# LMCache/LMCache

Hardware: NVIDIA B200
Metric: kv_encode_decode_raw_GBps (higher is better)
Workload: dtype f32->u8 (bf16 KV)

## Files before the change

lmcache_b200/csrc/codec.cu:

```cuda
#include <cuda_bf16.h>
#include <cuda_fp16.h>
#include <cuda_runtime.h>
#include <stdint.h>
#include <stdlib.h>

#include "ac_core.cuh"
#include "common.cuh"

namespace b200kv {

constexpr int CT = 128;
constexpr int SPW = 6;
constexpr int SYMW = 43;
constexpr int PAIRW = 33;
constexpr int TEMPW_FUSED = 40;
constexpr int TEMPW_SPLIT = 132;
constexpr int TEMPW_FUSED_RANS = 48;
constexpr int CODER_AC = 0, CODER_RANS = 1;
constexpr int CODER_RANS_COMPACT = 2;
constexpr int kHdrRowWords = 8;
constexpr int TEMPW_FUSED_RANS_HDR = TEMPW_FUSED_RANS + kHdrRowWords;

struct EncParams {
    PlaneTable pt;
    int64_t sT, sH, tok_begin;
    const int64_t* slot_map;
    int32_t L, H, D, C, dtype;
    int32_t n_chunks, chunk_tokens, last_chunk_tokens, tpp;
    int32_t tiles_full, tempw;
    int32_t stage_bytes;
    int32_t coder;
    int32_t compact;
    uint8_t* out;
    int64_t out_stride;
    uint64_t* sizes_out;
    uint32_t* temp;
    uint32_t* rstate;
    uint32_t* tile_tot;
    unsigned long long* totals;
    unsigned int* err;
};

template <class Prm>
__device__ __forceinline__ Layout layout_of(const Prm& P, int t) {
    return make_layout(P.L, P.C, t, P.compact);
}

__device__ __forceinline__ uint32_t load_len(const uint8_t* sec, int64_t idx, bool compact) {
    return compact ? 2u * (uint32_t)sec[idx] : (uint32_t)reinterpret_cast<const int32_t*>(sec)[idx];
}
__device__ __forceinline__ void store_len(uint8_t* sec, int64_t idx, uint32_t len, bool compact) {
    if (compact) sec[idx] = (uint8_t)(len >> 1);
    else reinterpret_cast<int32_t*>(sec)[idx] = (int32_t)len;
}

__device__ __forceinline__ uint32_t build_stream_header(const uint32_t (&cnt)[32], uint32_t mask, uint32_t wany, int nb,
                                                        uint32_t* rowfront, uint32_t& w0, uint32_t& w1) {
    const uint32_t top = 0x80000000u >> __clz((int)mask);
    const uint32_t st = mask & ~top;
    const uint32_t mb = (uint32_t)hdr_mask_bytes(nb);
    w0 = 0u;
    w1 = 0u;
    uint32_t widx = 0u, acc = mask, sh = 8u * mb;
    auto flush = [&]() {
        if (widx == 0u) w0 = acc;
        else if (widx == 1u) w1 = acc;
        else rowfront[widx - 2u] = acc;
        ++widx;
        acc = 0u;
        sh = 0u;
    };
    if (sh == 32u) flush();
#pragma unroll
    for (int i = 0; i < 32; ++i) {
        if (i < nb && ((wany >> i) & 1u) && ((st >> i) & 1u)) {
            acc |= cnt[i] << sh;
            sh += 8u;
            if (sh == 32u) flush();
        }
    }
    uint32_t hlen = mb + (uint32_t)__popc(st);
    hlen += hlen & 1u;
    if (sh != 0u) flush();
    return hlen;
}

__device__ __forceinline__ uint32_t read_header_mask(const uint8_t* p, int nb) {
    uint32_t m = *reinterpret_cast<const uint16_t*>(p);
    if (nb > 16) m |= (uint32_t)*reinterpret_cast<const uint16_t*>(p + 2) << 16;
    if (nb <= 8) m &= 0xffu;
    return nb >= 32 ? m : m & ((1u << nb) - 1u);
}

__device__ __forceinline__ int chunk_tokens_of(const EncParams& P, int j) {
    return j == P.n_chunks - 1 ? P.last_chunk_tokens : P.chunk_tokens;
}

template <bool PAGED>
__device__ __forceinline__ int64_t tok_row(const int64_t* slot_map, int64_t tok) {
    if constexpr (PAGED) return __ldg(slot_map + tok);
    else return tok;
}

template <bool VEC, bool PAGED>
__global__ void __launch_bounds__(256) absmax_kernel(EncParams P, int64_t total_tokens) {
    const int64_t warp = (blockIdx.x * (int64_t)blockDim.x + threadIdx.x) >> 5;
    const int lane = threadIdx.x & 31;
    const int64_t nrows = (int64_t)2 * P.L * total_tokens;
    if (warp >= nrows) return;
    const int nl = (int)(warp / total_tokens);
    const int64_t T = warp % total_tokens;
    const uint16_t* row = P.pt.p[nl] + tok_row<PAGED>(P.slot_map, P.tok_begin + T) * P.sT;
    uint32_t m = 0;
    if (VEC) {
        const int vec_per_head = P.D >> 3;
        const int nvec = P.H * vec_per_head;
        for (int v = lane; v < nvec; v += 32) {
            const int h = v / vec_per_head, dv = v - h * vec_per_head;
            const uint4 q = __ldg(reinterpret_cast<const uint4*>(row + (int64_t)h * P.sH + dv * 8));
            const uint32_t w[4] = {q.x, q.y, q.z, q.w};
#pragma unroll
            for (int k = 0; k < 4; ++k) {
                const uint32_t a = w[k] & 0x7fff7fffu;
                m = max(m, max(a & 0xffffu, a >> 16));
            }
        }
    } else {
        for (int c = lane; c < P.C; c += 32) {
            const int h = c / P.D, d = c - h * P.D;
            m = max(m, (uint32_t)(__ldg(row + (int64_t)h * P.sH + d) & 0x7fffu));
        }
    }
    m = __reduce_max_sync(0xffffffffu, m);
    if (lane == 0) {
        const int j = (int)(T / P.chunk_tokens);
        const int tj = chunk_tokens_of(P, j);
        const Layout lo = layout_of(P, tj);
        uint16_t* maxes = reinterpret_cast<uint16_t*>(P.out + (int64_t)j * P.out_stride + lo.off_maxes);
        maxes[(int64_t)nl * tj + (T - (int64_t)j * P.chunk_tokens)] = (uint16_t)m;
    }
}

__device__ __forceinline__ uint32_t block_excl_scan(uint32_t v, uint32_t* s_warp, uint32_t* total) {
    const int lane = threadIdx.x & 31, wid = threadIdx.x >> 5;
    uint32_t inc = v;
#pragma unroll
    for (int o = 1; o < 32; o <<= 1) {
        uint32_t n = __shfl_up_sync(0xffffffffu, inc, o);
        if (lane >= o) inc += n;
    }
    if (lane == 31) s_warp[wid] = inc;
    __syncthreads();
    uint32_t base = 0, tot = 0;
#pragma unroll
    for (int w = 0; w < CT / 32; ++w) {
        const uint32_t s = s_warp[w];
        if (w < wid) base += s;
        tot += s;
    }
    *total = tot;
    return base + inc - v;
}

struct TileId { int j, g, nl, ct, t, tok0, gt, tile_in_chunk; };
__device__ __forceinline__ bool decode_tile(const EncParams& P, uint32_t tile, TileId* id) {
    const uint32_t per_group = 2u * P.L * P.tpp;
    const uint32_t j = tile / (uint32_t)P.tiles_full;
    const uint32_t rem = tile - j * (uint32_t)P.tiles_full;
    id->j = (int)j;
    id->tile_in_chunk = (int)rem;
    id->t = chunk_tokens_of(P, (int)j);
    id->g = (int)(rem / per_group);
    if (id->g * kGroup >= id->t) return false;
    const uint32_t rem2 = rem - (uint32_t)id->g * per_group;
    id->nl = (int)(rem2 / P.tpp);
    id->ct = (int)(rem2 - (uint32_t)id->nl * P.tpp);
    id->tok0 = id->g * kGroup;
    id->gt = min(kGroup, id->t - id->tok0);
    return true;
}

template <int DT, bool PAGED, int BT, class F>
__device__ __forceinline__ void for_each_symbol(const uint16_t* cbase, const int64_t* slot_map, int64_t tokabs, int64_t s1,
                                                int gt, const float* fac, float maxq, F&& f) {
    const int nbatch = (gt + BT - 1) / BT;
    uint16_t xa[BT], xb[BT];
    auto load = [&](uint16_t (&x)[BT], int b) {
        const int tk = b * BT;
#pragma unroll
        for (int k = 0; k < BT; ++k)
            x[k] = tk + k < gt ? __ldg(cbase + tok_row<PAGED>(slot_map, tokabs + tk + k) * s1) : (uint16_t)0;
    };
    auto use = [&](const uint16_t (&x)[BT], int b) {
        const int tk = b * BT;
        uint32_t q[BT];
#pragma unroll
        for (int k = 0; k < BT; ++k) q[k] = quant_symbol(half_to_float(x[k], DT), fac[min(tk + k, kGroup - 1)], maxq);
#pragma unroll
        for (int k = 0; k < BT; ++k)
            if (tk + k < gt) f(q[k]);
    };
    load(xa, 0);
    for (int b = 0; b < nbatch; b += 2) {
        if (b + 1 < nbatch) load(xb, b + 1);
        use(xa, b);
        if (b + 1 < nbatch) {
            if (b + 2 < nbatch) load(xa, b + 2);
            use(xb, b + 1);
        }
    }
}

template <int DT, bool PAGED, int BT, class F>
__device__ __forceinline__ void for_each_symbol_rev(const uint16_t* cbase, const int64_t* slot_map, int64_t tokabs, int64_t s1,
                                                    int gt, const float* fac, float maxq, F&& f) {
    const int nbatch = (gt + BT - 1) / BT;
    uint16_t xa[BT], xb[BT];
    auto load = [&](uint16_t (&x)[BT], int b) {
        const int tk = b * BT;
#pragma unroll
        for (int k = 0; k < BT; ++k)
            x[k] = tk + k < gt ? __ldg(cbase + tok_row<PAGED>(slot_map, tokabs + tk + k) * s1) : (uint16_t)0;
    };
    auto use = [&](const uint16_t (&x)[BT], int b) {
        const int tk = b * BT;
        uint32_t q[BT];
#pragma unroll
        for (int k = 0; k < BT; ++k) q[k] = quant_symbol(half_to_float(x[k], DT), fac[min(tk + k, kGroup - 1)], maxq);
#pragma unroll
        for (int k = BT - 1; k >= 0; --k)
            if (tk + k < gt) f(q[k]);
    };
    load(xa, nbatch - 1);
    for (int b = nbatch - 1; b >= 0; b -= 2) {
        if (b >= 1) load(xb, b - 1);
        use(xa, b);
        if (b >= 1) {
            if (b >= 2) load(xa, b - 2);
            use(xb, b - 1);
        }
    }
}

__device__ __forceinline__ void rans_put(uint32_t& x, int32_t& nk, const uint16_t* row_end, uint32_t start, uint32_t freq) {
    const uint32_t xh = x >> 16;
    asm volatile(
        "{\n\t.reg .pred p;\n\t.reg .b64 ad;\n\t"
        "setp.ge.u32 p, %2, %3;\n\t"
        "mad.wide.s32 ad, %1, 2, %4;\n\t"
        "@p st.global.u16 [ad+-2], %0;\n\t"
        "@p add.s32 %1, %1, -1;\n\t"
        "selp.b32 %0, %2, %0, p;\n\t"
        "}"
        : "+r"(x), "+r"(nk) : "r"(xh), "r"(freq), "l"(row_end) : "memory");
    float rc;
    asm("rcp.approx.ftz.f32 %0, %1;" : "=f"(rc) : "f"(__uint2float_rn(freq)));
    const uint32_t q = __float2uint_rz(__uint2float_rz(x) * (rc * 0.99999952316284179688f));
    const uint32_t m = 65536u - freq;
    const uint32_t a = q * m + x;
    const uint32_t r = a - (q << 16);
    x = a + start;
    if (r >= freq) x += m;
}

template <bool FUSED, int DT, bool PAGED, int CODER>
__global__ void __launch_bounds__(CT, FUSED ? 7 : 4) encode_kernel(EncParams P) {
    extern __shared__ __align__(16) uint32_t smem[];
    constexpr int ROWS_W = FUSED ? CT * SYMW : 0;
    constexpr int TAB_W = FUSED ? (CT * kLp * 2 + 3) / 4 : CT * PAIRW;
    uint32_t* rows = smem;
    uint32_t* tab = smem + ROWS_W;
    float* fac = reinterpret_cast<float*>(smem + ((ROWS_W + TAB_W + 3) & ~3));
    __shared__ uint32_t s_warp[CT / 32];

    const int tid = threadIdx.x;
    TileId id;
    if (!decode_tile(P, blockIdx.x, &id)) return;
    const int NL = 2 * P.L;
    const int j = id.j, nl = id.nl, ct = id.ct, t = id.t, gt = id.gt;
    const int c = ct * CT + tid;
    const bool active = c < P.C;
    const int ncols = min(CT, P.C - ct * CT);

    uint8_t* cont = P.out + (int64_t)j * P.out_stride;
    const Layout lo = layout_of(P, t);
    const uint16_t* maxes = reinterpret_cast<const uint16_t*>(cont + lo.off_maxes) + (int64_t)nl * t + id.tok0;
    const float maxq = P.pt.maxq[nl];
    const int64_t s1 = P.sT;
    for (int i = tid; i < gt; i += CT)
        fac[i] = FUSED ? quant_factor_safe(maxq, half_to_float(maxes[i], DT)) : quant_factor(maxq, half_to_float(maxes[i], DT));
    if (FUSED) for (int i = gt + tid; i < kGroup + 8; i += CT) fac[i] = 0.0f;

    const int h = active ? c / P.D : 0;
    const int64_t tokabs = P.tok_begin + (int64_t)j * P.chunk_tokens + id.tok0;
    const uint16_t* cbase = P.pt.p[nl] + (int64_t)h * P.sH + (active ? c - h * P.D : 0);
    const uint16_t* src = cbase + (PAGED ? 0 : tokabs * P.sT);
    uint32_t* trow = P.temp + ((int64_t)blockIdx.x * CT + tid) * P.tempw;
    uint32_t cap = (uint32_t)P.tempw;
    asm volatile("" : "+l"(trow), "+r"(cap));
    uint32_t len = 0u, hlen = 0u;

    if (FUSED) {
        uint32_t* myrow = rows + tid * SYMW;
        uint16_t* cdfr = reinterpret_cast<uint16_t*>(tab);
        uint16_t* crow = cdfr + tid * kLp;
        uint16_t* hist = crow;
#pragma unroll
        for (int i = 0; i < kLp; ++i) crow[i] = 0;
        if (!PAGED) {
            const int lines_per_tok = (ncols * 2 + 127) >> 7;
            const uint16_t* tile0 = P.pt.p[nl] + (P.tok_begin + (int64_t)j * P.chunk_tokens + id.tok0) * P.sT +
                                    (int64_t)((ct * CT) / P.D) * P.sH + ((ct * CT) % P.D);
            if ((ct * CT) / P.D == (ct * CT + ncols - 1) / P.D)
                for (int i = tid; i < gt * lines_per_tok; i += CT) {
                    const int tok = i / lines_per_tok, ln = i - tok * lines_per_tok;
                    asm volatile("prefetch.global.L2 [%0];" ::"l"(tile0 + (int64_t)tok * s1 + ln * 64));
                }
        }
        __syncthreads();
        if (active) {
            constexpr int NB = 2, BT = NB * SPW;
            const int nbatch = (gt + BT - 1) / BT;
            uint16_t xa[BT], xb[BT];
            const uint32_t s1u = (uint32_t)s1;
            const uint32_t two = 2u * (uint32_t)min(P.n_chunks, 1);
            auto load = [&](uint16_t (&x)[BT], int b) {
                const int tk = b * BT;
                if constexpr (PAGED) {
                    const int64_t* sm = P.slot_map + tokabs + tk;
#pragma unroll
                    for (int k = 0; k < BT; ++k) x[k] = tk + k < gt ? __ldg(cbase + __ldg(sm + k) * s1) : (uint16_t)0;
                } else {
                    const uint16_t* q = src + (int64_t)tk * s1;
                    if (tk + BT <= gt) {
#pragma unroll
                        for (int k = 0; k < BT; ++k) {
                            x[k] = __ldg(q);
                            asm("mad.wide.u32 %0, %1, %2, %0;" : "+l"(q) : "r"(s1u), "r"(two));
                        }
                    } else {
#pragma unroll
                        for (int k = 0; k < BT; ++k) {
                            x[k] = tk + k < gt ? __ldg(q) : (uint16_t)0;
                            asm("mad.wide.u32 %0, %1, %2, %0;" : "+l"(q) : "r"(s1u), "r"(two));
                        }
                    }
                }
            };
            auto quantise = [&](const uint16_t (&x)[BT], int b) {
                const int tk = b * BT;
                uint32_t q[BT];
#pragma unroll
                for (int k = 0; k < BT; ++k) q[k] = quant_symbol_nc(half_to_float(x[k], DT), fac[tk + k], maxq);
#pragma unroll
                for (int half = 0; half < NB; ++half) {
                    if (tk + half * SPW < gt) {
                        uint32_t word = 0u;
#pragma unroll
                        for (int k = 0; k < SPW; ++k) {
                            hist[q[half * SPW + k]] += 1;
                            word |= q[half * SPW + k] << (5 * k);
                        }
                        myrow[b * NB + half] = word;
                    }
                }
            };
            load(xa, 0);
            for (int b = 0; b < nbatch; b += 2) {
                if (b + 1 < nbatch) load(xb, b + 1);
                quantise(xa, b);
                if (b + 1 < nbatch) {
                    if (b + 2 < nbatch) load(xa, b + 2);
                    quantise(xb, b + 1);
                }
            }
            const int pad = (gt + SPW - 1) / SPW * SPW - gt;
            if (pad) hist[quant_symbol(0.0f, 0.0f, maxq)] -= (uint16_t)pad;
        }
        __syncthreads();
        {
            const float tf = (float)t;
            for (int n = tid; n <= t; n += CT) fac[n] = fdiv((float)n, tf);
        }
        __syncthreads();
        if (active) {
            uint32_t cnt[32];
#pragma unroll
            for (int i = 0; i < 32; ++i) cnt[i] = hist[i];
            uint32_t mask = 0u;
#pragma unroll
            for (int i = 0; i < 32; ++i) mask |= (cnt[i] != 0u ? 1u : 0u) << i;
            const uint32_t wany = __reduce_or_sync(__activemask(), mask);
            CdfAccum2 acc;
            acc.init();
#pragma unroll
            for (uint32_t i = 0; i < 32u; ++i) {
                crow[i] = (uint16_t)acc.value(i);
                if ((wany >> i) & 1u) acc.absorb(fac[cnt[i]]);
            }
            crow[32] = (uint16_t)acc.value(32u);
            if (P.compact) {
                uint32_t w0, w1;
                hlen = build_stream_header(cnt, mask, wany, 2 * ((int)maxq + 1), trow, w0, w1);
                reinterpret_cast<uint2*>(P.rstate)[((int64_t)blockIdx.x * CT + tid) * 2] = make_uint2(w0, w1);
            }
        }
        __syncthreads();
        if (!P.compact) {
            uint16_t* dstc = reinterpret_cast<uint16_t*>(cont + lo.off_cdf) + ((int64_t)nl * P.C + ct * CT) * kLp;
            for (int e = tid; e < ncols * kLp; e += CT) dstc[e] = cdfr[e];
        }
        if (active && CODER == CODER_RANS) {
            uint32_t x = kRansLow;
            const uint16_t* const wend = reinterpret_cast<const uint16_t*>(trow) + 2 * P.tempw;
            int32_t nk = 0;
            const char* const cb = reinterpret_cast<const char*>(crow);
            auto code = [&](uint32_t word, int k) {
                const uint32_t o = (k == 0 ? word << 1 : word >> (5 * k - 1)) & 62u;
                const uint32_t c_lo = *reinterpret_cast<const uint16_t*>(cb + o);
                const uint32_t c_hi = *reinterpret_cast<const uint16_t*>(cb + o + 2);
                rans_put(x, nk, wend, c_lo, c_hi - c_lo);
            };
            int w = (gt - 1) / SPW;
            {
                const uint32_t word = myrow[w];
                for (int k = gt - 1 - w * SPW; k >= 0; --k) code(word, k);
            }
            for (--w; w >= 0; --w) {
                const uint32_t word = myrow[w];
#pragma unroll
                for (int k = SPW - 1; k >= 0; --k) code(word, k);
            }
            if (P.compact) reinterpret_cast<uint2*>(P.rstate)[((int64_t)blockIdx.x * CT + tid) * 2 + 1] = make_uint2(x, hlen);
            else P.rstate[(int64_t)blockIdx.x * CT + tid] = x;
            len = hlen + 4u - 2u * (uint32_t)nk;
        } else if (active) {
            EncState2 st;
            st.init();
            int tk = 0;
            for (int w = 0; tk < gt; ++w) {
                const uint32_t word = myrow[w];
                if (tk + SPW <= gt) {
#pragma unroll
                    for (int k = 0; k < SPW; ++k) {
                        const uint32_t sidx = (word >> (5 * k)) & 31u;
                        const uint32_t c_lo = crow[sidx];
                        enc_symbol2(st, c_lo, (uint32_t)crow[sidx + 1u] - c_lo, trow, cap);
                    }
                    tk += SPW;
                } else {
                    for (int k = 0; tk < gt; ++k, ++tk) {
                        const uint32_t sidx = (word >> (5 * k)) & 31u;
                        const uint32_t c_lo = crow[sidx];
                        enc_symbol2(st, c_lo, (uint32_t)crow[sidx + 1u] - c_lo, trow, cap);
                    }
                }
            }
            len = enc_finish2(st, trow, cap);
            if (st.w > cap) atomicOr(&P.err[j], 1u);
        }
    } else {
        uint32_t* prow = tab + tid * PAIRW;
        const uint16_t* cdf_src =
            reinterpret_cast<const uint16_t*>(cont + lo.off_cdf) + ((int64_t)nl * P.C + ct * CT) * kLp;
        for (int e = tid; e < ncols * kLp; e += CT) tab[e] = cdf_src[e];
        __syncthreads();
        if (active) {
            uint32_t cv[kLp];
#pragma unroll
            for (int i = 0; i < kLp; ++i) cv[i] = prow[i] & 0xffffu;
#pragma unroll
            for (int i = 0; i < 32; ++i) {
                const uint32_t hi = (i == 31) ? 0x10000u : cv[i + 1];
                prow[i] = cv[i] | ((hi - cv[i]) << 16);
            }
            if (CODER == CODER_RANS) {
                uint32_t x = kRansLow;
                const uint16_t* const wend = reinterpret_cast<const uint16_t*>(trow) + 2 * TEMPW_SPLIT;
                int32_t nk = 0;
                for_each_symbol_rev<DT, PAGED, 4>(cbase, P.slot_map, tokabs, s1, gt, fac, maxq, [&](uint32_t q) {
                    const uint32_t pr = prow[q];
                    rans_put(x, nk, wend, pr & 0xffffu, pr >> 16);
                });
                P.rstate[(int64_t)blockIdx.x * CT + tid] = x;
                len = 4u - 2u * (uint32_t)nk;
            } else {
                EncState2 st;
                st.init();
                for_each_symbol<DT, PAGED, 4>(cbase, P.slot_map, tokabs, s1, gt, fac, maxq, [&](uint32_t q) {
                    const uint32_t pr = prow[q];
                    enc_symbol2(st, pr & 0xffffu, pr >> 16, trow, cap);
                });
                len = enc_finish2(st, trow, cap);
                if (st.w > cap) atomicOr(&P.err[j], 1u);
            }
        }
    }

    if (active) store_len(cont + lo.off_lengths, ((int64_t)id.g * NL + nl) * P.C + c, len, P.compact != 0);
    uint32_t tile_total;
    (void)block_excl_scan(len, s_warp, &tile_total);
// ... 845 lines not shown
    if (!active) return;
    const uint32_t* erow = tab + tid * kLp;
    const int h = c / P.D;
    uint16_t* dst = const_cast<uint16_t*>(P.pt.p[nl]) + (PAGED ? 0 : (dc.dst_tok + tok0) * P.sT) + (int64_t)h * P.sH +
                    (c - h * P.D);
    const int64_t* slots = PAGED ? P.slot_map + dc.dst_tok + tok0 : nullptr;
    uint32_t bad = beyond ? 2u : 0u;
    if constexpr (CODER == CODER_RANS) {
        uint32_t xf;
        const uint32_t one = min((uint32_t)P.n_chunks, 1u);
        const uint32_t* pk = TR ? tab + tid : tab + tid * kLp;
        if (cq <= 7.0f) xf = rans_decode_stream<OUT_DT, 4, PAGED, TR>(dc.base, my_off + hl, pk, lut, mx, dst, (uint32_t)P.sT, gt, slots, one);
        else xf = rans_decode_stream<OUT_DT, 5, PAGED, TR>(dc.base, my_off + hl, pk, lut, mx, dst, (uint32_t)P.sT, gt, slots, one);
        bad |= xf != kRansLow ? 1u : 0u;
    } else {
        if (cq <= 7.0f) decode_stream<OUT_DT, 4, PAGED>(dc.base, my_off, erow, lut, mx, dst, (uint32_t)P.sT, gt, slots);
        else decode_stream<OUT_DT, 5, PAGED>(dc.base, my_off, erow, lut, mx, dst, (uint32_t)P.sT, gt, slots);
    }
    if (bad != 0u && P.status != nullptr) atomicOr(&P.status[j], bad);
}

int make_plane_table(const b200kv_kv_desc* kv, const float* key_bins, const float* value_bins, PlaneTable* out) {
    B2_REQUIRE(kv != nullptr, "kv descriptor is NULL");
    B2_REQUIRE(kv->L > 0 && 2 * kv->L <= B200KV_MAX_PLANES, "L out of range");
    B2_REQUIRE(kv->H > 0 && kv->D > 0, "H/D must be positive");
    B2_REQUIRE(kv->dtype == B200KV_DT_BF16 || kv->dtype == B200KV_DT_FP16, "dtype must be bf16 or fp16");
    B2_REQUIRE(kv->planes != nullptr || kv->base != nullptr, "no KV pointer");
    for (int kvi = 0; kvi < 2; ++kvi)
        for (int l = 0; l < kv->L; ++l) {
            const int nl = kvi * kv->L + l;
            const uint16_t* p = kv->planes ? static_cast<const uint16_t*>(kv->planes[nl])
                                           : static_cast<const uint16_t*>(kv->base) + l * kv->sL + kvi * kv->sKV;
            B2_REQUIRE(p != nullptr, "NULL plane pointer");
            out->p[nl] = p;
            const float bins = kvi ? value_bins[l] : key_bins[l];
            out->maxq[nl] = floorf(bins / 2.0f) - 1.0f;
            B2_REQUIRE(out->maxq[nl] >= 1.0f && out->maxq[nl] <= 15.0f, "bins must be in [4, 32]");
        }
    return 0;
}

static int tiles_per_plane(int C) { return (C + CT - 1) / CT; }

enum { kProfAbsmax = 0, kProfCdf, kProfEncode, kProfFinalize, kProfTileSum, kProfTileScan, kProfDecode, kProfCount };
static bool g_prof_on = false;
static cudaEvent_t g_prof_ev[kProfCount][2];
static bool g_prof_have[kProfCount];
static bool g_prof_init = false;

struct ProfScope {
    int slot;
    cudaStream_t stream;
    ProfScope(int slot_, cudaStream_t s) : slot(slot_), stream(s) {
        if (!g_prof_on) return;
        if (!g_prof_init) {
            for (int i = 0; i < kProfCount; ++i) { cudaEventCreate(&g_prof_ev[i][0]); cudaEventCreate(&g_prof_ev[i][1]); }
            g_prof_init = true;
        }
        cudaEventRecord(g_prof_ev[slot][0], stream);
    }
    ~ProfScope() {
        if (!g_prof_on) return;
        cudaEventRecord(g_prof_ev[slot][1], stream);
        g_prof_have[slot] = true;
    }
};

static int enc_tempw(bool fused, int coder, bool compact = false) {
    if (compact) return TEMPW_FUSED_RANS_HDR;
    return fused ? (coder == CODER_RANS ? TEMPW_FUSED_RANS : TEMPW_FUSED) : TEMPW_SPLIT;
}

static size_t enc_ws_layout(int64_t n_tiles_alloc, int n_chunks, int tempw, int coder, bool compact, size_t* off_tot,
                            size_t* off_totals, size_t* off_err, size_t* off_state, size_t* off_temp) {
    size_t o = 0;
    *off_tot = o;    o += (size_t)n_tiles_alloc * 4;  o = (o + 255) & ~(size_t)255;
    *off_totals = o; o += (size_t)n_chunks * 8;       o = (o + 255) & ~(size_t)255;
    *off_err = o;    o += (size_t)n_chunks * 4;       o = (o + 255) & ~(size_t)255;
    *off_state = o;  o += coder == CODER_RANS ? (size_t)n_tiles_alloc * CT * (compact ? 16 : 4) : 0;  o = (o + 255) & ~(size_t)255;
    *off_temp = o;   o += (size_t)n_tiles_alloc * CT * (size_t)tempw * 4;
    return (o + 255) & ~(size_t)255;
}

static size_t dec_ws_layout(int64_t tiles_max, int n_chunks, size_t* off_tb) {
    size_t o = ((size_t)n_chunks * sizeof(DecChunk) + 255) & ~(size_t)255;
    *off_tb = o;
    o += (size_t)n_chunks * (size_t)tiles_max * 8;
    return (o + 255) & ~(size_t)255;
}

}

using namespace b200kv;

extern "C" {

int b200kv_container_layout(int32_t L, int32_t H, int32_t D, int32_t ntokens, b200kv_layout* out) {
    return b200kv_container_layout_v(L, H, D, ntokens, CODER_RANS, out);
}

int b200kv_container_layout_v(int32_t L, int32_t H, int32_t D, int32_t ntokens, int32_t coder, b200kv_layout* out) {
    B2_REQUIRE(out != nullptr && L > 0 && H > 0 && D > 0 && ntokens > 0, "bad shape");
    B2_REQUIRE(coder >= CODER_AC && coder <= CODER_RANS_COMPACT, "unknown coder");
    const int compact = coder == CODER_RANS_COMPACT ? 1 : 0;
    B2_REQUIRE(!compact || ntokens <= kGroup, "the compact container holds chunks of at most 256 tokens");
    const Layout lo = make_layout(L, H * D, ntokens, compact);
    out->off_cdf = lo.off_cdf;
    out->off_maxes = lo.off_maxes;
    out->off_lengths = lo.off_lengths;
    out->off_payload = lo.off_payload;
    out->fixed_bytes = lo.off_payload;
    const int64_t streams = 2 * (int64_t)L * H * D;
    out->max_total_bytes = align16(lo.off_payload + streams * (2 * (int64_t)ntokens + 4 * (int64_t)lo.ngroups +
                                                              (compact ? kHdrMax : 0)) + 16);
    return 0;
}

int64_t b200kv_encode_workspace_bytes(int32_t L, int32_t H, int32_t D, int32_t chunk_tokens, int32_t n_chunks,
                                      int32_t coder) {
    if (L <= 0 || H <= 0 || D <= 0 || chunk_tokens <= 0 || n_chunks <= 0) return -2;
    coder &= 0xff;
    const bool compact = coder == CODER_RANS_COMPACT;
    if (compact) coder = CODER_RANS;
    if (coder != CODER_AC && coder != CODER_RANS) return -2;
    if (compact && chunk_tokens > kGroup) return -2;
    const int64_t G = (chunk_tokens + kGroup - 1) / kGroup;
    const int64_t n_tiles = (int64_t)n_chunks * G * 2 * L * tiles_per_plane(H * D);
    size_t a, b, c, d, e;
    return (int64_t)enc_ws_layout(n_tiles, n_chunks, enc_tempw(chunk_tokens <= kGroup, coder, compact), coder, compact, &a, &b, &c, &d, &e);
}

int64_t b200kv_decode_workspace_bytes(int32_t L, int32_t H, int32_t D, int32_t chunk_tokens, int32_t n_chunks) {
    if (L <= 0 || H <= 0 || D <= 0 || chunk_tokens <= 0 || n_chunks <= 0) return -2;
    const int64_t G = (chunk_tokens + kGroup - 1) / kGroup;
    const int64_t tiles_max = G * 2 * L * tiles_per_plane(H * D);
    size_t a;
    return (int64_t)dec_ws_layout(tiles_max, n_chunks, &a);
}

int b200kv_encode_chunks(const b200kv_kv_desc* kv, int64_t tok_begin, int32_t n_chunks, int32_t chunk_tokens,
                         int32_t last_chunk_tokens, const float* key_bins, const float* value_bins, int32_t coder,
                         void* out, int64_t out_stride, uint64_t* sizes_out, void* workspace, int64_t workspace_bytes,
                         void* stream_) {
    cudaStream_t stream = static_cast<cudaStream_t>(stream_);
    EncParams P;
    B2_REQUIRE(key_bins && value_bins, "bins are NULL");
    const bool hint_tma = (coder & B200KV_ENCODE_HINT_HIGH_ENTROPY) != 0;
    const bool hint_mid = (coder & B200KV_ENCODE_HINT_MID_ENTROPY) != 0;
    coder &= 0xff;
    B2_REQUIRE(coder >= CODER_AC && coder <= CODER_RANS_COMPACT, "coder must be one of B200KV_CODER_*");
    P.compact = coder == CODER_RANS_COMPACT ? 1 : 0;
    if (P.compact) coder = CODER_RANS;
    P.coder = coder;
    if (int rc = make_plane_table(kv, key_bins, value_bins, &P.pt)) return rc;
    B2_REQUIRE(n_chunks > 0 && chunk_tokens > 0, "n_chunks / chunk_tokens must be positive");
    B2_REQUIRE(!P.compact || chunk_tokens <= kGroup, "the compact container (B200KV_CODER_RANS_COMPACT) holds chunks of at most 256 tokens");
    B2_REQUIRE(last_chunk_tokens > 0 && last_chunk_tokens <= chunk_tokens, "last_chunk_tokens out of range");
    B2_REQUIRE(out != nullptr && (reinterpret_cast<uintptr_t>(out) & 15) == 0 && (out_stride & 15) == 0,
               "out / out_stride must be 16-byte aligned");
    B2_REQUIRE(tok_begin >= 0, "tok_begin must be >= 0");
    P.sT = kv->sT; P.sH = kv->sH; P.tok_begin = tok_begin;
    P.slot_map = kv->slot_map;
    const bool paged = kv->slot_map != nullptr;
    P.L = kv->L; P.H = kv->H; P.D = kv->D; P.C = kv->H * kv->D; P.dtype = kv->dtype;
    P.n_chunks = n_chunks; P.chunk_tokens = chunk_tokens; P.last_chunk_tokens = last_chunk_tokens;
    P.tpp = tiles_per_plane(P.C);
    P.out = static_cast<uint8_t*>(out);
    P.out_stride = out_stride;
    P.sizes_out = sizes_out;
    const Layout lo = make_layout(P.L, P.C, chunk_tokens, P.compact);
    B2_REQUIRE(out_stride >= lo.off_payload + 16, "out_stride smaller than the fixed container sections");

    const int64_t G = lo.ngroups;
    const int64_t per_group = 2 * (int64_t)P.L * P.tpp;
    const int64_t tiles_full = G * per_group;
    const int64_t n_tiles = (int64_t)n_chunks * tiles_full;
    const bool fused = chunk_tokens <= kGroup;
    P.tiles_full = (int32_t)tiles_full;
    P.tempw = enc_tempw(fused, coder, P.compact != 0);
    size_t off_tot, off_totals, off_err, off_state, off_temp;
    const size_t need = enc_ws_layout(n_tiles, n_chunks, P.tempw, coder, P.compact != 0, &off_tot, &off_totals, &off_err, &off_state,
                                      &off_temp);
    B2_REQUIRE(workspace != nullptr && workspace_bytes >= (int64_t)need, "workspace too small");
    B2_REQUIRE(n_tiles < (1ll << 31) && tiles_full < (1ll << 31), "too many tiles in one call");
    uint8_t* ws = static_cast<uint8_t*>(workspace);
    P.tile_tot = reinterpret_cast<uint32_t*>(ws + off_tot);
    P.totals = reinterpret_cast<unsigned long long*>(ws + off_totals);
    P.err = reinterpret_cast<unsigned int*>(ws + off_err);
    P.temp = reinterpret_cast<uint32_t*>(ws + off_temp);
    P.rstate = reinterpret_cast<uint32_t*>(ws + off_state);
    B2_CHECK_CUDA(cudaMemsetAsync(ws, 0, off_state, stream));

    const int64_t total_tokens = (int64_t)(n_chunks - 1) * chunk_tokens + last_chunk_tokens;
    for (int i = 0; i <= kProfFinalize; ++i) g_prof_have[i] = false;
    {
        bool vec = (kv->D % 8 == 0) && (kv->sT % 8 == 0) && (kv->sH % 8 == 0);
        for (int nl = 0; nl < 2 * P.L && vec; ++nl) vec = (reinterpret_cast<uintptr_t>(P.pt.p[nl]) & 15) == 0;
        const int64_t rows = 2 * (int64_t)P.L * total_tokens;
        const int64_t blocks = (rows + 7) / 8;
        B2_REQUIRE(blocks < (1ll << 31), "too many rows in one call");
        ProfScope prof(kProfAbsmax, stream);
        if (vec && !paged) absmax_kernel<true, false><<<(unsigned)blocks, 256, 0, stream>>>(P, total_tokens);
        else if (vec) absmax_kernel<true, true><<<(unsigned)blocks, 256, 0, stream>>>(P, total_tokens);
        else if (!paged) absmax_kernel<false, false><<<(unsigned)blocks, 256, 0, stream>>>(P, total_tokens);
        else absmax_kernel<false, true><<<(unsigned)blocks, 256, 0, stream>>>(P, total_tokens);
        B2_CHECK_CUDA(cudaGetLastError());
    }
    const size_t smem_fused = (size_t)(((CT * SYMW + (CT * kLp * 2 + 3) / 4 + 3) & ~3) + kGroup + 8) * 4;
    const size_t smem_split = (size_t)(((CT * PAIRW + 3) & ~3) + kGroup + 4) * 4;
    const size_t smem_cdf = (size_t)(CT * PAIRW + kGroup) * 4;
#define B2_LAUNCH_ENC1(FUSED, DT, PAGED, CODER, SMEM)                                                      \
    do {                                                                                                   \
        B2_CHECK_CUDA(cudaFuncSetAttribute(encode_kernel<FUSED, DT, PAGED, CODER>,                         \
                                           cudaFuncAttributeMaxDynamicSharedMemorySize, (int)(SMEM)));     \
        encode_kernel<FUSED, DT, PAGED, CODER><<<(unsigned)n_tiles, CT, (SMEM), stream>>>(P);              \
    } while (0)
#define B2_LAUNCH_ENC(FUSED, DT, PAGED, SMEM)                                                              \
    do {                                                                                                   \
        if (coder == CODER_RANS) B2_LAUNCH_ENC1(FUSED, DT, PAGED, CODER_RANS, SMEM);                       \
        else B2_LAUNCH_ENC1(FUSED, DT, PAGED, CODER_AC, SMEM);                                             \
    } while (0)
#define B2_LAUNCH_ENC2(FUSED, SMEM)                                                                        \
    do {                                                                                                   \
        if (P.dtype == B200KV_DT_BF16) { if (paged) B2_LAUNCH_ENC(FUSED, 0, true, SMEM); else B2_LAUNCH_ENC(FUSED, 0, false, SMEM); } \
        else { if (paged) B2_LAUNCH_ENC(FUSED, 1, true, SMEM); else B2_LAUNCH_ENC(FUSED, 1, false, SMEM); } \
    } while (0)
    bool tma = hint_tma;
    if (const char* e = getenv("B200KV_ENCODE_PATH")) tma = e[0] == 't';
    tma = tma && fused && coder == CODER_RANS && P.C % CT == 0 && (kv->sH == kv->D || kv->D % CT == 0) &&
          kv->sT % 8 == 0 && kv->sH % 8 == 0;
    for (int nl = 0; nl < 2 * P.L && tma; ++nl) tma = (reinterpret_cast<uintptr_t>(P.pt.p[nl]) & 15) == 0;
    if (tma) {
        ProfScope prof(kProfEncode, stream);
#define B2_LAUNCH_TMA(DT, PAGED)                                                                                       \
    do {                                                                                                               \
        B2_CHECK_CUDA(cudaFuncSetAttribute(encode_tma_kernel<DT, PAGED>, cudaFuncAttributeMaxDynamicSharedMemorySize,  \
                                           kEncTmaSmem));                                                              \
        encode_tma_kernel<DT, PAGED><<<(unsigned)n_tiles, CT, kEncTmaSmem, stream>>>(P);                               \
    } while (0)
        if (P.dtype == B200KV_DT_BF16) { if (paged) B2_LAUNCH_TMA(0, true); else B2_LAUNCH_TMA(0, false); }
        else { if (paged) B2_LAUNCH_TMA(1, true); else B2_LAUNCH_TMA(1, false); }
#undef B2_LAUNCH_TMA
    } else if (fused) {
        ProfScope prof(kProfEncode, stream);
        B2_LAUNCH_ENC2(true, smem_fused);
    } else {
        const unsigned cdf_blocks = (unsigned)((int64_t)n_chunks * per_group);
        {
            ProfScope prof(kProfCdf, stream);
            if (P.dtype == B200KV_DT_BF16) {
                if (paged) cdf_kernel<0, true><<<cdf_blocks, CT, smem_cdf, stream>>>(P);
                else cdf_kernel<0, false><<<cdf_blocks, CT, smem_cdf, stream>>>(P);
            } else {
                if (paged) cdf_kernel<1, true><<<cdf_blocks, CT, smem_cdf, stream>>>(P);
                else cdf_kernel<1, false><<<cdf_blocks, CT, smem_cdf, stream>>>(P);
            }
        }
        B2_CHECK_CUDA(cudaGetLastError());
        ProfScope prof(kProfEncode, stream);
        B2_LAUNCH_ENC2(false, smem_split);
    }
#undef B2_LAUNCH_ENC2
#undef B2_LAUNCH_ENC
#undef B2_LAUNCH_ENC1
    B2_CHECK_CUDA(cudaGetLastError());
    {
        ProfScope prof(kProfFinalize, stream);
        P.stage_bytes = coder == CODER_RANS ? CT * (TEMPW_FUSED_RANS * 4 + 4) + 32 : CT * TEMPW_FUSED * 4 + 32;
        if (coder == CODER_RANS && !hint_tma && !hint_mid) P.stage_bytes = 12 * 1024;
        if (const char* e = getenv("B200KV_COMPACT_STAGE")) {
            const int v = atoi(e);
            if (v >= 1024 && v <= P.stage_bytes + 16 * 1024) P.stage_bytes = v & ~15;
        }
        B2_CHECK_CUDA(cudaFuncSetAttribute(compact_kernel, cudaFuncAttributeMaxDynamicSharedMemorySize, P.stage_bytes));
        enc_scan_kernel<<<(unsigned)n_chunks, 1024, 0, stream>>>(P);
        compact_kernel<<<(unsigned)n_tiles, CT, (size_t)P.stage_bytes, stream>>>(P);
        finalize_kernel<<<(n_chunks + 127) / 128, 128, 0, stream>>>(P);
    }
    B2_CHECK_CUDA(cudaGetLastError());
    return 0;
}

int b200kv_decode_chunks(const void* containers, int64_t containers_bytes, const int64_t* offsets,
                         const int64_t* total_bytes, const int32_t* ntokens, const int64_t* dst_tok, int32_t n_chunks,
                         int32_t max_dtype,
                         int32_t coder, const b200kv_kv_desc* dst, const float* key_bins, const float* value_bins,
                         uint32_t* status_out, void* workspace, int64_t workspace_bytes, void* stream_) {
    cudaStream_t stream = static_cast<cudaStream_t>(stream_);
    DecParams P;
    B2_REQUIRE(key_bins && value_bins, "bins are NULL");
    B2_REQUIRE(coder >= CODER_AC && coder <= CODER_RANS_COMPACT, "coder must be one of B200KV_CODER_*");
    P.compact = coder == CODER_RANS_COMPACT ? 1 : 0;
    if (P.compact) coder = CODER_RANS;
    if (int rc = make_plane_table(dst, key_bins, value_bins, &P.pt)) return rc;
    B2_REQUIRE(containers && offsets && total_bytes && ntokens && dst_tok && n_chunks > 0, "bad chunk arrays");
    B2_REQUIRE(max_dtype == B200KV_DT_BF16 || max_dtype == B200KV_DT_FP16, "bad max_dtype");
    B2_REQUIRE(dst->sT > 0 && dst->sT < (1ll << 23), "destination token stride out of range");
    P.sT = dst->sT; P.sH = dst->sH;
    P.slot_map = dst->slot_map;
    P.L = dst->L; P.H = dst->H; P.D = dst->D; P.C = dst->H * dst->D;
    P.out_dtype = dst->dtype; P.max_dtype = max_dtype; P.n_chunks = n_chunks;
    P.tpp = tiles_per_plane(P.C);
    int tmax = 0;
    for (int j = 0; j < n_chunks; ++j) {
        B2_REQUIRE(ntokens[j] > 0, "ntokens must be positive");
        B2_REQUIRE(!P.compact || ntokens[j] <= kGroup, "a compact container holds at most 256 tokens");
        B2_REQUIRE((offsets[j] & 15) == 0, "container offsets must be 16-byte aligned");
        const Layout lj = make_layout(P.L, P.C, ntokens[j], P.compact);
        B2_REQUIRE(total_bytes[j] >= lj.off_payload && total_bytes[j] - lj.off_payload < (1ll << 32),
                   "container shorter than its fixed sections (truncated or corrupt)");
        B2_REQUIRE(offsets[j] >= 0 && offsets[j] + total_bytes[j] + B200KV_READ_SLACK <= containers_bytes,
                   "containers buffer must extend B200KV_READ_SLACK bytes past the end of every container");
        tmax = ntokens[j] > tmax ? ntokens[j] : tmax;
    }
    const int64_t Gmax = (tmax + kGroup - 1) / kGroup;
    const int64_t tiles_max = Gmax * 2 * P.L * P.tpp;
    B2_REQUIRE(tiles_max < (1ll << 31) && n_chunks <= 65535, "too many tiles / chunks in one call");
    bool transposed = false;
    {
        double bits = 0.0, syms = 0.0;
        for (int j = 0; j < n_chunks; ++j) {
            const Layout lj = make_layout(P.L, P.C, ntokens[j], P.compact);
            bits += 8.0 * (double)(total_bytes[j] - lj.off_payload);
            syms += 2.0 * P.L * (double)P.C * ntokens[j];
        }
        transposed = bits > (P.compact ? 4.1 : 3.6) * syms && bits < 6.0 * syms;
        if (const char* e = getenv("B200KV_DECODE_TABLE")) transposed = e[0] == 't';
    }
    P.tiles_max = (int32_t)tiles_max;
    size_t off_tb;
    const size_t need = dec_ws_layout(tiles_max, n_chunks, &off_tb);
    B2_REQUIRE(workspace != nullptr && workspace_bytes >= (int64_t)need, "workspace too small");
    uint8_t* ws = static_cast<uint8_t*>(workspace);
    {
        DecChunk* hc = static_cast<DecChunk*>(malloc(sizeof(DecChunk) * (size_t)n_chunks));
        B2_REQUIRE(hc != nullptr, "out of host memory");
        for (int j = 0; j < n_chunks; ++j) {
            hc[j].base = static_cast<const uint8_t*>(containers) + offsets[j];
            hc[j].dst_tok = dst_tok[j];
            hc[j].t = ntokens[j];
            hc[j].ngroups = (ntokens[j] + kGroup - 1) / kGroup;
            const Layout lj = make_layout(P.L, P.C, ntokens[j], P.compact);
            hc[j].payload_bytes = (uint32_t)(total_bytes[j] - lj.off_payload);
            hc[j].pad = 0;
        }
        cudaError_t e = cudaMemcpyAsync(ws, hc, sizeof(DecChunk) * (size_t)n_chunks, cudaMemcpyHostToDevice, stream);
        free(hc);
        B2_CHECK_CUDA(e);
    }
    P.chunks = reinterpret_cast<const DecChunk*>(ws);
    P.tile_base = reinterpret_cast<unsigned long long*>(ws + off_tb);
    P.status = status_out;
    if (status_out) B2_CHECK_CUDA(cudaMemsetAsync(status_out, 0, sizeof(uint32_t) * (size_t)n_chunks, stream));

    dim3 gsum((unsigned)((tiles_max + 3) / 4), (unsigned)n_chunks);
    {
        ProfScope prof(kProfTileSum, stream);
        tile_sum_kernel<<<gsum, 128, 0, stream>>>(P);
    }
    B2_CHECK_CUDA(cudaGetLastError());
    {
// ... 48 lines not shown
```

Before: 542.2.

## Add 4-bit packed nibble fast path for compact rANS encode

Adds a specialised fused-encode path for the compact rANS coder when the quantisation range fits in 15 symbols. Symbols are packed 8 per word as 4-bit nibbles in a column-major shared layout, histograms are built with shared atomic adds, and per-symbol reciprocals are precomputed so the rANS step skips its per-symbol rcp. This aims to cut shared-memory traffic and ALU work in the encode loop. In exchange the fused kernel's shared-memory request may grow, there is a new branch, and an A/B script is added.

Measured after the change: 557.1, median of 6. 1.03x the previous value.

```diff
diff --git a/lmcache_b200/csrc/codec.cu b/lmcache_b200/csrc/codec.cu
--- a/lmcache_b200/csrc/codec.cu
+++ b/lmcache_b200/csrc/codec.cu
@@ -3,6 +3,7 @@
 #include <cuda_runtime.h>
 #include <stdint.h>
 #include <stdlib.h>
+#include <string.h>
 
 #include "ac_core.cuh"
 #include "common.cuh"
@@ -12,6 +13,11 @@
 constexpr int CT = 128;
 constexpr int SPW = 6;
 constexpr int SYMW = 43;
+constexpr int SPW4 = 8;
+constexpr int NSYM16 = 15;
+constexpr int NB16_TAB_W = 32 * CT;
+constexpr int NB16_RCP_W = NB16_TAB_W + NSYM16 * CT;
+constexpr int NB16_SMEM_W = NB16_RCP_W + NSYM16 * CT;
 constexpr int PAIRW = 33;
 constexpr int TEMPW_FUSED = 40;
 constexpr int TEMPW_SPLIT = 132;
@@ -39,6 +45,7 @@
     uint32_t* tile_tot;
     unsigned long long* totals;
     unsigned int* err;
+    int32_t nb16;
 };
 
 template <class Prm>
@@ -242,7 +249,15 @@
     }
 }
 
-__device__ __forceinline__ void rans_put(uint32_t& x, int32_t& nk, const uint16_t* row_end, uint32_t start, uint32_t freq) {
+constexpr float kRcpBias = 0.99999952316284179688f;
+__device__ __forceinline__ float rans_rcp(uint32_t freq) {
+    float rc;
+    asm("rcp.approx.ftz.f32 %0, %1;" : "=f"(rc) : "f"(__uint2float_rn(freq)));
+    return rc * kRcpBias;
+}
+template <bool RC_GIVEN>
+__device__ __forceinline__ void rans_step(uint32_t& x, int32_t& nk, const uint16_t* row_end, uint32_t start, uint32_t freq,
+                                          float rc_given) {
     const uint32_t xh = x >> 16;
     asm volatile(
         "{\n\t.reg .pred p;\n\t.reg .b64 ad;\n\t"
@@ -253,14 +268,26 @@
         "selp.b32 %0, %2, %0, p;\n\t"
         "}"
         : "+r"(x), "+r"(nk) : "r"(xh), "r"(freq), "l"(row_end) : "memory");
-    float rc;
-    asm("rcp.approx.ftz.f32 %0, %1;" : "=f"(rc) : "f"(__uint2float_rn(freq)));
-    const uint32_t q = __float2uint_rz(__uint2float_rz(x) * (rc * 0.99999952316284179688f));
+    uint32_t q;
+    if constexpr (RC_GIVEN) {
+        q = __float2uint_rz(__uint2float_rz(x) * rc_given);
+    } else {
+        float rc;
+        asm("rcp.approx.ftz.f32 %0, %1;" : "=f"(rc) : "f"(__uint2float_rn(freq)));
+        q = __float2uint_rz(__uint2float_rz(x) * (rc * kRcpBias));
+    }
     const uint32_t m = 65536u - freq;
     const uint32_t a = q * m + x;
     const uint32_t r = a - (q << 16);
     x = a + start;
     if (r >= freq) x += m;
+}
+__device__ __forceinline__ void rans_put(uint32_t& x, int32_t& nk, const uint16_t* row_end, uint32_t start, uint32_t freq) {
+    rans_step<false>(x, nk, row_end, start, freq, 0.0f);
+}
+__device__ __forceinline__ void rans_put_rc(uint32_t& x, int32_t& nk, const uint16_t* row_end, uint32_t start, uint32_t freq,
+                                            float rc) {
+    rans_step<true>(x, nk, row_end, start, freq, rc);
 }
 
 template <bool FUSED, int DT, bool PAGED, int CODER>
@@ -300,53 +327,168 @@
     asm volatile("" : "+l"(trow), "+r"(cap));
     uint32_t len = 0u, hlen = 0u;
 
-    if (FUSED) {
+    constexpr int BT = 12;
+    const uint32_t s1u = (uint32_t)s1;
+    const uint32_t two = 2u * (uint32_t)min(P.n_chunks, 1);
+    auto load = [&](uint16_t (&x)[BT], int b) {
+        const int tk = b * BT;
+        if constexpr (PAGED) {
+            const int64_t* sm = P.slot_map + tokabs + tk;
+#pragma unroll
+            for (int k = 0; k < BT; ++k) x[k] = tk + k < gt ? __ldg(cbase + __ldg(sm + k) * s1) : (uint16_t)0;
+        } else {
+            const uint16_t* q = src + (int64_t)tk * s1;
+            if (tk + BT <= gt) {
+#pragma unroll
+                for (int k = 0; k < BT; ++k) {
+                    x[k] = __ldg(q);
+                    asm("mad.wide.u32 %0, %1, %2, %0;" : "+l"(q) : "r"(s1u), "r"(two));
+                }
+            } else {
+#pragma unroll
+                for (int k = 0; k < BT; ++k) {
+                    x[k] = tk + k < gt ? __ldg(q) : (uint16_t)0;
+                    asm("mad.wide.u32 %0, %1, %2, %0;" : "+l"(q) : "r"(s1u), "r"(two));
+                }
+            }
+        }
+    };
+    if (FUSED && !PAGED) {
+        const int lines_per_tok = (ncols * 2 + 127) >> 7;
+        const uint16_t* tile0 = P.pt.p[nl] + (P.tok_begin + (int64_t)j * P.chunk_tokens + id.tok0) * P.sT +
+                                (int64_t)((ct * CT) / P.D) * P.sH + ((ct * CT) % P.D);
+        if ((ct * CT) / P.D == (ct * CT + ncols - 1) / P.D)
+            for (int i = tid; i < gt * lines_per_tok; i += CT) {
+                const int tok = i / lines_per_tok, ln = i - tok * lines_per_tok;
+                asm volatile("prefetch.global.L2 [%0];" ::"l"(tile0 + (int64_t)tok * s1 + ln * 64));
+            }
+    }
+
+    if (FUSED && CODER == CODER_RANS && P.nb16 && maxq <= 7.0f) {
+        static_assert(CT * 4 == 1 << 9, "pass 2 forms symbol * CT * 4 with a shift by 9");
+        static_assert(!FUSED || (((ROWS_W + TAB_W + 3) & ~3) >= NB16_RCP_W &&
+                                 ((ROWS_W + TAB_W + 3) & ~3) + kGroup + 8 <= NB16_SMEM_W), "fac must lie inside rcp");
+        uint32_t* const wcol = smem + tid;
+        uint32_t* const tcol = smem + NB16_TAB_W + tid;
+        const uint32_t tcol_a = (uint32_t)__cvta_generic_to_shared(tcol);
+#pragma unroll
+        for (int s = 0; s < NSYM16; ++s) tcol[s * CT] = 0u;
+        __syncthreads();
+        if (active) {
+            const int nbatch = (gt + BT - 1) / BT;
+            uint16_t xa[BT], xb[BT];
+            uint32_t carry = 0u;
+            auto quantise = [&](const uint16_t (&x)[BT], int b, bool odd) {
+                const int tk = b * BT;
+                uint32_t q[BT];
+#pragma unroll
+                for (int k = 0; k < BT; ++k) q[k] = quant_symbol_nc(half_to_float(x[k], DT), fac[tk + k], maxq);
+#pragma unroll
+                for (int k = 0; k < BT; ++k)
+                    asm volatile("red.shared.add.u32 [%0], 1;" ::"r"(tcol_a + q[k] * (CT * 4)) : "memory");
+                uint32_t* const wp = wcol + (tk / SPW4) * CT;
+                if (!odd) {
+                    uint32_t w0 = 0u;
+#pragma unroll
+                    for (int k = 0; k < SPW4; ++k) w0 |= q[k] << (4 * k);
+                    wp[0] = w0;
+                    carry = 0u;
+#pragma unroll
+                    for (int k = SPW4; k < BT; ++k) carry |= q[k] << (4 * (k - SPW4));
+                } else {
+                    uint32_t w1 = carry;
+#pragma unroll
+                    for (int k = 0; k < BT - SPW4; ++k) w1 |= q[k] << (4 * (k + BT - SPW4));
+                    wp[0] = w1;
+                    if (tk + BT - SPW4 < gt) {
+                        uint32_t w2 = 0u;
+#pragma unroll
+                        for (int k = 0; k < SPW4; ++k) w2 |= q[BT - SPW4 + k] << (4 * k);
+                        wp[CT] = w2;
+                    }
+                }
+            };
+            load(xa, 0);
+            for (int b = 0; b < nbatch; b += 2) {
+                if (b + 1 < nbatch) load(xb, b + 1);
+                quantise(xa, b, false);
+                if (b + 1 < nbatch) {
+                    if (b + 2 < nbatch) load(xa, b + 2);
+                    quantise(xb, b + 1, true);
+                }
+            }
+            if ((nbatch & 1) && (nbatch - 1) * BT + SPW4 < gt) wcol[((nbatch - 1) * BT / SPW4 + 1) * CT] = carry;
+            tcol[quant_symbol(0.0f, 0.0f, maxq) * CT] -= (uint32_t)(nbatch * BT - gt);
+        }
+        __syncthreads();
+        {
+            const float tf = (float)t;
+            for (int n = tid; n <= t; n += CT) fac[n] = fdiv((float)n, tf);
+        }
+        __syncthreads();
+        if (active) {
+            uint32_t cnt[32];
+#pragma unroll
+            for (int i = 0; i < 32; ++i) cnt[i] = i < NSYM16 ? tcol[i * CT] : 0u;
+            uint32_t mask = 0u;
+#pragma unroll
+            for (int i = 0; i < NSYM16; ++i) mask |= (cnt[i] != 0u ? 1u : 0u) << i;
+            const uint32_t wany = __reduce_or_sync(__activemask(), mask);
+            uint32_t w0, w1;
+            hlen = build_stream_header(cnt, mask, wany, 2 * ((int)maxq + 1), trow, w0, w1);
+            reinterpret_cast<uint2*>(P.rstate)[((int64_t)blockIdx.x * CT + tid) * 2] = make_uint2(w0, w1);
+            CdfAccum2 acc;
+            acc.init();
+            uint32_t c0 = 0u;
+#pragma unroll
+            for (uint32_t i = 0; i < (uint32_t)NSYM16; ++i) {
+                if ((wany >> i) & 1u) acc.absorb(fac[cnt[i]]);
+                const uint32_t c1 = acc.value(i + 1u);
+                tcol[i * CT] = c0 | ((c1 - c0) << 16);
+                c0 = c1;
+            }
+        }
+        __syncthreads();
+        if (active) {
+            float* const rcol = reinterpret_cast<float*>(smem + NB16_RCP_W) + tid;
+#pragma unroll
+            for (int s = 0; s < NSYM16; ++s) rcol[s * CT] = rans_rcp(tcol[s * CT] >> 16);
+            uint32_t x = kRansLow;
+            const uint16_t* const wend = reinterpret_cast<const uint16_t*>(trow) + 2 * P.tempw;
+            int32_t nk = 0;
+            const char* const tb = reinterpret_cast<const char*>(smem + NB16_TAB_W);
+            const char* const rb = reinterpret_cast<const char*>(smem + NB16_RCP_W);
+            const uint32_t tid4 = 4u * (uint32_t)tid;
+            auto code = [&](uint32_t word, int k) {
+                const uint32_t o = ((4 * k >= 9 ? word >> (4 * k - 9) : word << (9 - 4 * k)) & (15u << 9)) | tid4;
+                const uint32_t pk = *reinterpret_cast<const uint32_t*>(tb + o);
+                rans_put_rc(x, nk, wend, pk & 0xffffu, pk >> 16, *reinterpret_cast<const float*>(rb + o));
+            };
+            int w = (gt - 1) / SPW4;
+            {
+                const uint32_t word = wcol[w * CT];
+                for (int k = gt - 1 - w * SPW4; k >= 0; --k) code(word, k);
+            }
+            for (--w; w >= 0; --w) {
+                const uint32_t word = wcol[w * CT];
+#pragma unroll
+                for (int k = SPW4 - 1; k >= 0; --k) code(word, k);
+            }
+            reinterpret_cast<uint2*>(P.rstate)[((int64_t)blockIdx.x * CT + tid) * 2 + 1] = make_uint2(x, hlen);
+            len = hlen + 4u - 2u * (uint32_t)nk;
+        }
+    } else if (FUSED) {
         uint32_t* myrow = rows + tid * SYMW;
         uint16_t* cdfr = reinterpret_cast<uint16_t*>(tab);
         uint16_t* crow = cdfr + tid * kLp;
         uint16_t* hist = crow;
 #pragma unroll
         for (int i = 0; i < kLp; ++i) crow[i] = 0;
-        if (!PAGED) {
-            const int lines_per_tok = (ncols * 2 + 127) >> 7;
-            const uint16_t* tile0 = P.pt.p[nl] + (P.tok_begin + (int64_t)j * P.chunk_tokens + id.tok0) * P.sT +
-                                    (int64_t)((ct * CT) / P.D) * P.sH + ((ct * CT) % P.D);
-            if ((ct * CT) / P.D == (ct * CT + ncols - 1) / P.D)
-                for (int i = tid; i < gt * lines_per_tok; i += CT) {
-                    const int tok = i / lines_per_tok, ln = i - tok * lines_per_tok;
-                    asm volatile("prefetch.global.L2 [%0];" ::"l"(tile0 + (int64_t)tok * s1 + ln * 64));
-                }
-        }
         __syncthreads();
         if (active) {
-            constexpr int NB = 2, BT = NB * SPW;
+            constexpr int NB = BT / SPW;
             const int nbatch = (gt + BT - 1) / BT;
             uint16_t xa[BT], xb[BT];
-            const uint32_t s1u = (uint32_t)s1;
-            const uint32_t two = 2u * (uint32_t)min(P.n_chunks, 1);
-            auto load = [&](uint16_t (&x)[BT], int b) {
-                const int tk = b * BT;
-                if constexpr (PAGED) {
-                    const int64_t* sm = P.slot_map + tokabs + tk;
-#pragma unroll
-                    for (int k = 0; k < BT; ++k) x[k] = tk + k < gt ? __ldg(cbase + __ldg(sm + k) * s1) : (uint16_t)0;
-                } else {
-                    const uint16_t* q = src + (int64_t)tk * s1;
-                    if (tk + BT <= gt) {
-#pragma unroll
-                        for (int k = 0; k < BT; ++k) {
-                            x[k] = __ldg(q);
-                            asm("mad.wide.u32 %0, %1, %2, %0;" : "+l"(q) : "r"(s1u), "r"(two));
-                        }
-                    } else {
-#pragma unroll
-                        for (int k = 0; k < BT; ++k) {
-                            x[k] = tk + k < gt ? __ldg(q) : (uint16_t)0;
-                            asm("mad.wide.u32 %0, %1, %2, %0;" : "+l"(q) : "r"(s1u), "r"(two));
-                        }
-                    }
-                }
-            };
             auto quantise = [&](const uint16_t (&x)[BT], int b) {
                 const int tk = b * BT;
                 uint32_t q[BT];
@@ -1498,6 +1640,8 @@
     P.compact = coder == CODER_RANS_COMPACT ? 1 : 0;
     if (P.compact) coder = CODER_RANS;
     P.coder = coder;
+    P.nb16 = P.compact;
+    if (const char* e = getenv("B200KV_ENCODE_NB16")) P.nb16 = P.nb16 && strcmp(e, "off") != 0;
     if (int rc = make_plane_table(kv, key_bins, value_bins, &P.pt)) return rc;
     B2_REQUIRE(n_chunks > 0 && chunk_tokens > 0, "n_chunks / chunk_tokens must be positive");
     B2_REQUIRE(!P.compact || chunk_tokens <= kGroup, "the compact container (B200KV_CODER_RANS_COMPACT) holds chunks of at most 256 tokens");
@@ -1552,7 +1696,8 @@
         else absmax_kernel<false, true><<<(unsigned)blocks, 256, 0, stream>>>(P, total_tokens);
         B2_CHECK_CUDA(cudaGetLastError());
     }
-    const size_t smem_fused = (size_t)(((CT * SYMW + (CT * kLp * 2 + 3) / 4 + 3) & ~3) + kGroup + 8) * 4;
+    const size_t smem_fused5 = (size_t)(((CT * SYMW + (CT * kLp * 2 + 3) / 4 + 3) & ~3) + kGroup + 8) * 4;
+    const size_t smem_fused = smem_fused5 > (size_t)NB16_SMEM_W * 4 ? smem_fused5 : (size_t)NB16_SMEM_W * 4;
     const size_t smem_split = (size_t)(((CT * PAIRW + 3) & ~3) + kGroup + 4) * 4;
     const size_t smem_cdf = (size_t)(CT * PAIRW + kGroup) * 4;
 #define B2_LAUNCH_ENC1(FUSED, DT, PAGED, CODER, SMEM)                                                      \
diff --git a/profiles/nb16_ab.py b/profiles/nb16_ab.py
--- /dev/null
+++ b/profiles/nb16_ab.py
@@ -0,0 +1,105 @@
+#!/usr/bin/env python
+import argparse
+import ctypes
+import json
+import os
+import statistics
+import subprocess
+import sys
+
+ROOT = os.path.dirname(os.path.dirname(os.path.abspath(__file__)))
+sys.path.insert(0, ROOT)
+import torch
+
+import __graft_entry__ as ge
+from bench import L, H, D, MODEL, synth_kv_torch
+
+ge.build_cuda()
+from lmcache_b200 import _native as N
+from lmcache_b200.codec import CacheGenCodec, KvView
+
+ap = argparse.ArgumentParser()
+ap.add_argument("--rounds", type=int, default=7)
+ap.add_argument("--steps", type=int, default=5, help="passes over the 8192-token block per setting and round")
+args = ap.parse_args()
+
+torch.cuda.set_device(0)
+dev = torch.device("cuda", 0)
+T, cs, W = 8192, 256, 8
+kv = synth_kv_torch(T, dev, 1234 + 2, "kv8d")
+view = KvView.from_blob(kv, "vllm")
+codec = CacheGenCodec(MODEL)
+stride = codec.out_stride(L, H, D, cs)
+buf = torch.empty(stride * W + N.READ_SLACK, dtype=torch.uint8, device=dev)
+lib = N.lib()
+enc_slot = N.PROFILE_SLOTS.index("encode")
+os.environ["B200KV_ENCODE_PATH"] = "legacy"
+
+
+def setting(name):
+    if name == "off":
+        os.environ["B200KV_ENCODE_NB16"] = "off"
+    else:
+        os.environ.pop("B200KV_ENCODE_NB16", None)
+
+
+def waves(steps):
+    kern, call = [], []
+    prof = (ctypes.c_float * 8)()
+    lib.b200kv_profile_enable(1)
+    for _ in range(steps):
+        for c0 in range(0, T // cs, W):
+            e0, e1 = torch.cuda.Event(enable_timing=True), torch.cuda.Event(enable_timing=True)
+            e0.record()
+            codec.encode_async(view, c0 * cs, W * cs, cs, out=buf)
+            e1.record()
+            torch.cuda.synchronize()
+            N.check(lib.b200kv_profile_last(prof, 8))
+            kern.append(prof[enc_slot])
+            call.append(e0.elapsed_time(e1))
+    lib.b200kv_profile_enable(0)
+    return kern, call
+
+
+same = True
+ref = None
+for name in ("off", "on"):
+    setting(name)
+    codec.encode_async(view, 0, W * cs, cs, out=buf).wait()
+    b = buf.clone()
+    same = same and (ref is None or torch.equal(b, ref))
+    ref = b
+
+for name in ("off", "on"):
+    setting(name)
+    waves(2)
+per = {"off": {"kernel": [], "call": []}, "on": {"kernel": [], "call": []}}
+for r in range(args.rounds):
+    for name in (("off", "on") if r % 2 == 0 else ("on", "off")):
+        setting(name)
+        k, c = waves(args.steps)
+        per[name]["kernel"].append(statistics.median(k))
+        per[name]["call"].append(statistics.median(c))
+
+
+def summary(v):
+    m = statistics.median(v)
+    return {"median_ms": round(m, 4), "min_ms": round(min(v), 4), "max_ms": round(max(v), 4),
+            "spread_pct": round(100.0 * (max(v) - min(v)) / m, 2), "per_round_ms": [round(x, 4) for x in v]}
+
+
+gpu = {"name": torch.cuda.get_device_name(0)}
+try:
+    q = subprocess.run(["nvidia-smi", "--query-gpu=power.limit,clocks.max.sm", "--format=csv,noheader", "-i", "0"],
+                       capture_output=True, text=True, timeout=30).stdout.strip()
+    gpu["power_limit_and_max_sm_clock"] = q
+except (OSError, subprocess.SubprocessError):
+    pass
+res = {"workload": f"{L}L/{H}H/{D}D, {T} tokens kv8d, chunk {cs}, container v3, waves of {W} chunks",
+       "gpu": gpu, "rounds": args.rounds, "waves_per_round": args.steps * T // (cs * W),
+       "containers_identical": bool(same),
+       "encode_kernel_per_wave": {k: summary(per[k]["kernel"]) for k in per},
+       "encode_call_per_wave": {k: summary(per[k]["call"]) for k in per}}
+res["encode_kernel_speedup"] = round(res["encode_kernel_per_wave"]["off"]["median_ms"] /
+                                     res["encode_kernel_per_wave"]["on"]["median_ms"], 4)
+print(json.dumps(res))
```
